# sjin09/himut

Hardware: AMD Instinct MI355X
Metric: Mbp scanned/sec at 30x CCS (himut call pileup scan) (higher is better)
Workload: dtype u8/int32 + f64 genotype tail; 1 GPU; chr20-sized contig (64444167 bp) 30x synthetic CCS per GPU, common-SNP + PoN filtering, reference chunking (323 chunks); reads_per_gpu=128888, read_bases_per_gpu=1932346823, parallelism=contig-per-gpu x1 + RCCL gather

## Files before the change

### himut_amd/csrc/himut_call.hip

```cpp
#include <hip/hip_runtime.h>

#include <string.h>
#include <rocprim/rocprim.hpp>

#include "himut_ctx.h"
#include "himut_kernels.h"
#include "himut_reads.h"

using namespace himut;

namespace himut {


namespace {

struct ParseSide {
    const Params* P = nullptr;
    uint32_t* bits = nullptr;
    int64_t nwords = 0;
    void* fill = nullptr;
    int64_t fill_slots = 0;
};

void ensure_group_plan(himut_ctx* c) {
// ... 252 lines not shown
    A.counts = c->call.d_dense_counts.as<uint32_t>(); A.bqsum = c->call.d_dense_bqsum.as<uint32_t>(); A.err = err;
    hipLaunchKernelGGL((k_pile_dense<PD_TP, PD_RB, PD_NT>), dim3((unsigned)T.n_tiles), dim3(PD_NT), 0, st, A);
}


void call_reserve_records(himut_ctx* c, CallPlan* P) {
    himut_ctx::Call& K = c->call;
    const int64_t nreserve = P->nreserve;
    K.d_recs.reserve((size_t)(nreserve + 1) * sizeof(himut_record));
    K.d_recs_out.reserve((size_t)(nreserve + 1) * sizeof(himut_record));
    if (P->ncap <= 0) return;
    K.d_keys.reserve((size_t)nreserve * 8); K.d_keys2.reserve((size_t)nreserve * 8);
    K.d_cands.reserve((size_t)nreserve * sizeof(Cand) + 256); K.d_cands2.reserve((size_t)nreserve * sizeof(Cand) + 256);
    K.d_emit.reserve((size_t)nreserve * 4);
    if (!c->chunks_in_order) {
        HCHECK(rocprim::radix_sort_pairs(nullptr, P->sort_tmp, K.d_keys.as<uint64_t>(), K.d_keys2.as<uint64_t>(), K.d_cands.as<uint64_t>(),
                                         K.d_cands2.as<uint64_t>(), (size_t)P->ncap, 0, 60, c->stream));
        c->d_tmp.reserve(P->sort_tmp + 256);
    }
    const unsigned nb = blocks_for(P->ncap, 256);
    K.d_logpart.reserve((size_t)nb * 16 * 4 + 64);
    K.d_pos.reserve((size_t)nb * 4 + 64);
}

int call_plan(himut_ctx* c, bool allow_spec, CallPlan* P) {
    himut_ctx::Call& K = c->call;
    P->T = upload_chunks(c, c->cstart, c->cend);
    P->phase = c->params.p.phase != 0;
    P->spec = allow_spec && c->chunks_in_order && K.cap_cand > 0 && K.cap_slots > 0 && P->T.positions > 0 && c->n > 0;
    alloc_derived(c);
    P->n4 = ((int64_t)P->T.positions * 2 + 15) / 16;
    P->mask_bytes = (size_t)P->n4 * 16;
    P->anyw = ((int64_t)P->T.positions + 31) / 32;
    P->mtiles = blocks_for(P->anyw, 256);
    const uint64_t mask_was = K.d_mask.gen;
    K.d_mask.reserve(P->mask_bytes + 64);
    const bool clear_mask = !K.mask_clean || mask_was != K.d_mask.gen;
    K.mask_clean = false;
    const uint64_t tcnt_was = K.d_tilecnt.gen;
    K.d_tilecnt.reserve((size_t)P->mtiles * 4 + 64);
    K.d_tileoff2.reserve((size_t)P->mtiles * 4 + 64);
    P->clear_all = clear_mask || tcnt_was != K.d_tilecnt.gen;
    if (P->phase && P->T.n > 65535) return fail(c, HIMUT_ERR_ARG, "--phase: more than 65,535 chunks in one contig (k_read_hap takes a chunk per grid row)");
    if (P->phase) c->d_hap.reserve((size_t)P->T.npairs + 64);
    P->F = front_plan(c, P->spec, K.cap_slots);
    if (P->mtiles > 65536u) {
        uint32_t* nul = nullptr;
        HCHECK(rocprim::exclusive_scan(nullptr, P->scan_tiles, nul, nul, 0u, (size_t)P->mtiles, rocprim::plus<uint32_t>(), c->stream));
    }
    c->d_tmp2.reserve(P->scan_tiles + 256);
    if (P->spec) {
        P->ncap = P->nreserve = K.cap_cand;
        call_reserve_records(c, P);
    }
    return HIMUT_OK;
}

int call_candidates(himut_ctx* c, CallPlan* P, const Chunks& C) {
    hipStream_t st = c->stream;
    himut_ctx::Call& K = c->call;
    Scalars* sc = c->d_scalars.as<Scalars>();
    uint32_t *tilecnt = K.d_tilecnt.as<uint32_t>(), *tileoff = K.d_tileoff2.as<uint32_t>();
    if (P->anyw > 0) {
        if (P->mtiles <= 65536u)
            hipLaunchKernelGGL(k_scan_small, dim3(1), dim3(1024), 0, st, tilecnt, tileoff, (int)P->mtiles);
        else
            HCHECK(rocprim::exclusive_scan(c->d_tmp2.p, P->scan_tiles, tilecnt, tileoff, 0u, (size_t)P->mtiles, rocprim::plus<uint32_t>(), st));
    }
    if (!P->spec) {
        uint32_t last_tcnt = 0, last_toff = 0;
        if (P->anyw > 0) {
            HCHECK(hipMemcpyAsync(&last_tcnt, tilecnt + (P->mtiles - 1), 4, hipMemcpyDeviceToHost, st));
            HCHECK(hipMemcpyAsync(&last_toff, tileoff + (P->mtiles - 1), 4, hipMemcpyDeviceToHost, st));
        }
        HCHECK(hipMemcpyAsync(c->h_scalars, sc, sizeof(Scalars), hipMemcpyDeviceToHost, st));
        HCHECK(hipStreamSynchronize(st));
        if (const int err = reinterpret_cast<const Scalars*>(c->h_scalars)->err) return check_device_err(c, err);
        P->ncap = (int64_t)last_toff + last_tcnt;
        P->nreserve = P->ncap + P->ncap / 4 + 1024;
        call_reserve_records(c, P);
    }
    if (P->ncap > 0) {
        const bool sorted = c->chunks_in_order;
        hipLaunchKernelGGL(k_mask_emit, dim3(P->mtiles), dim3(256), 0, st, K.d_posbits_c.as<uint32_t>(), (int64_t)P->T.positions,
                           K.d_mask.as<uint16_t>(), tileoff, C, (sorted ? K.d_cands2 : K.d_cands).as<Cand>(),
                           (sorted ? K.d_keys2 : K.d_keys).as<uint64_t>(), P->ncap, &sc->ncand, tilecnt);
        if (!sorted)
            HCHECK(rocprim::radix_sort_pairs(c->d_tmp.p, P->sort_tmp, K.d_keys.as<uint64_t>(), K.d_keys2.as<uint64_t>(), K.d_cands.as<uint64_t>(),
                                             K.d_cands2.as<uint64_t>(), (size_t)P->ncap, 0, 60, st));
    }
    stage_event(c, EV_EMIT, 2, st);
    return HIMUT_OK;
}

void call_eval(himut_ctx* c, const CallPlan& P, const Reads& R, const Derived& D, const Chunks& C, const Phase& H) {
    Scalars* sc = c->d_scalars.as<Scalars>();
    if (P.ncap > 0) {
        EvalArgs A;
        A.P = c->params;
        A.S = site_sets(c);
        A.lut = c->d_lut.as<GtLut>();
        A.cands = c->call.d_cands2.as<Cand>(); A.ncand = P.ncap; A.ncand_dev = &sc->ncand;
        A.R = R; A.D = D; A.C = C; A.H = H; A.X = P.F.X;
        A.colstore = c->call.d_colstore.as<uint16_t>(); A.nslots = (int64_t)P.F.slot_cap;
        A.recs = c->call.d_recs.as<himut_record>();
        A.err = &sc->err;
        hipLaunchKernelGGL(P.phase ? k_eval_columns<true> : k_eval_columns<false>, dim3(blocks_for(P.ncap, 256)), dim3(256), 0, c->stream, A);
    }
    stage_event(c, EV_SWEEP, 2, c->stream);
}

void call_finalize(himut_ctx* c, const CallPlan& P) {
    hipStream_t st = c->stream;
    himut_ctx::Call& K = c->call;
    Scalars* sc = c->d_scalars.as<Scalars>();
    if (P.ncap > 0) {
        const unsigned nb = blocks_for(P.ncap, 256);
        hipLaunchKernelGGL(k_finalize_flags, dim3(nb), dim3(256), 0, st, K.d_recs.as<himut_record>(), K.d_keys2.as<uint64_t>(),
                           &sc->ncand, P.ncap, K.d_emit.as<uint32_t>(), K.d_logpart.as<uint32_t>(),
                           c->d_ccs.as<uint8_t>(), c->n);
        hipLaunchKernelGGL(k_run_totals, dim3(1), dim3(1024), 0, st, P.ncap, K.d_blkoff.as<uint32_t>(), K.d_blkslots.as<uint32_t>(), P.F.nblk,
                           &sc->nrec, &sc->nslots, K.d_logpart.as<uint32_t>(), (int64_t)nb, sc->log, K.d_pos.as<uint32_t>());
        hipLaunchKernelGGL(k_compact, dim3(nb), dim3(256), 0, st, K.d_recs.as<himut_record>(), K.d_emit.as<uint32_t>(),
                           K.d_pos.as<uint32_t>(), &sc->ncand, P.ncap, K.d_recs_out.as<himut_record>());
    } else if (c->n > 0) {
        launch_count_flags(c, sc);
    }
}

int finish_run(himut_ctx* c, bool* overflow);

int do_run_once(himut_ctx* c, bool allow_spec, bool* overflow, bool defer) {
    *overflow = false;
    c->call.pending.active = false;
    if (int rc = check_scan_inputs(c)) return rc;
    HCHECK(hipSetDevice(c->device));
    c->call.h_recs_valid = false;
    c->call.n_out = 0;
    memset(c->call.log, 0, sizeof(c->call.log));
    memset(&c->stats, 0, sizeof(c->stats));
    c->params.unique_qnames = c->unique_qnames ? 1 : 0;

    CallPlan P;
    if (int rc = call_plan(c, allow_spec, &P)) return rc;
    const Reads R = make_reads(c);
    const Derived D = make_derived(c);
    const Chunks C = make_chunks(c, P.T.n);
    const Phase H = make_phase(c);
    front_decode(c, P.F, c->params, P.clear_all);
    if (P.phase && P.T.npairs > 0) launch_read_hap(c, R, D, C, H, P.T, c->d_scalars.as<Scalars>());
    stage_event(c, EV_HAP, 2, c->stream);
    if (int rc = front_capture(c, &P.F, C, H, c->params, c->call.d_mask.as<uint32_t>(), c->call.d_tilecnt.as<uint32_t>())) return rc;
    if (int rc = call_candidates(c, &P, C)) return rc;
    call_eval(c, P, R, D, C, H);
    call_finalize(c, P);
    front_tail(c, P.F);
    c->call.pending.active = true;
    c->call.pending.plan = P;
    if (defer) return HIMUT_OK;
    return finish_run(c, overflow);
}

int finish_run(himut_ctx* c, bool* overflow) {
    *overflow = false;
    const PendingRun Q = c->call.pending;
    c->call.pending.active = false;
    if (!Q.active) return HIMUT_OK;
    HCHECK(hipSetDevice(c->device));
// ... 177 lines not shown
```

### himut_amd/csrc/himut_kernels.h

```cpp
#pragma once

#include "himut_device.h"

namespace himut {

constexpr int EMIT_MAXC = 4;
constexpr int PROP_TAB_BITS = 11;

__device__ __forceinline__ void propose_read(const Reads& R, const Derived& D, const Chunks& C, const Phase& H, const Params& P,
                                             const int64_t r, const uint32_t bqs, const int e0, const int estride, const int gl,
                                             const int gsh, uint32_t* mask, uint32_t* tilecnt, uint8_t* ccs_flag,
                                             unsigned long long* s_seen) {
    auto propose = [&](const int64_t cell, const int bit) {
        if (s_seen) {
            const unsigned long long key = ((unsigned long long)cell << 4) | (unsigned long long)bit;
            const uint32_t h = (uint32_t)((key * 0x9E3779B97F4A7C15ull) >> (64 - PROP_TAB_BITS));
            if (atomicExch(&s_seen[h], key) == key) return;
        }
        const uint32_t m = (1u << bit) << ((cell & 1) ? 16 : 0);
        if (!(atomicOr(mask + (cell >> 1), m) & m)) atomicAdd(tilecnt + (cell >> MASK_TILE_SHIFT), 1u);
    };
#define GBALLOT(P) ((uint32_t)((__ballot(P) >> gsh) & 0xffffull))
    const ReadMeta M = D.meta[r];
    const int32_t qlen = R.qlen[r];
// ... 45 lines not shown
            for (int k = 0; k < EMIT_MAXC; k++) {
                if (rest) {
                    const int src = __ffs((int)rest) - 1;
                    rest &= rest - 1;
                    cc[k] = __shfl(rec.idx, src, 16); cst[k] = __shfl(rec.start, src, 16); cen[k] = __shfl(rec.end, src, 16);
                    cmo[k] = ((int64_t)__shfl((int)(rec.maskoff >> 32), src, 16) << 32) | (uint32_t)__shfl((int)rec.maskoff, src, 16);
                }
            }
        }
        if (nc == 0) live = false;
        else if (gl == 0) ccs_flag[qid] = 1;
    } else live = false;

    if (!live) return;
    const int32_t* mis = D.mis + M.segbase;
    const uint32_t* mq = D.mq + M.segbase;
    const double trim_start = floor(P.p.min_trim * (double)qlen);
    const double trim_end = ceil((1.0 - P.p.min_trim) * (double)qlen);
    const int64_t w = P.p.mismatch_window_size;
    for (int e = e0; e < nm; e += estride) {
        const uint32_t v = mq[e];
        const int32_t tp1 = mis[e];
        const int32_t mprev = e > 0 ? mis[e - 1] : -0x7fffffff - 1;
        const int32_t mnext = e + 1 < nm ? mis[e + 1] : 0x7fffffff;
        if (!(v & 16u)) continue;
        const int64_t q = v >> 5;
        if ((double)q < trim_start || (double)q > trim_end) continue;
        {
            int64_t qs = q - w, qe = q + w, ur, dr;
            if (qs < 0) { ur = w + qs; dr = w - qs; }
            else if (qe > qlen) { ur = w + (qe - qlen); dr = qlen - q; }
            else { ur = w; dr = w; }
            const int32_t ms = (int32_t)(tp1 - ur), me = (int32_t)(tp1 + dr);
            int lo = e, up = e + 1;
            if (mprev >= ms) { lo = e - 1; while (lo > 0 && mis[lo - 1] >= ms) lo--; }
            if (mnext <= me) { up = e + 2; while (up < nm && mis[up] <= me) up++; }
            if ((int64_t)(up - lo) - 1 > P.p.max_mismatch_count) continue;
        }
        const int bit = (int)(v & 15u);
        if (!overflow) {
#pragma unroll
            for (int k = 0; k < EMIT_MAXC; k++)
                if (cc[k] >= 0 && cst[k] <= tp1 && tp1 <= cen[k]) propose(cmo[k] + (tp1 - cst[k]), bit);
        } else {
            for (int64_t jj = hi - 1; jj >= 0 && C.rec[jj].pmaxend > ts; jj--) {
                const ChunkRec qr = C.rec[jj];
                if (qr.end <= ts || !(qr.start <= tp1 && tp1 <= qr.end)) continue;
                if (phase && H.hap[qr.pairbase + r] == HAP_NONE) continue;
                propose(qr.maskoff + (tp1 - qr.start), bit);
            }
        }
    }
#undef GBALLOT
}


struct CellCursor {
    int64_t ck, cbeg, cend;
    int32_t cstart;
};

__device__ __forceinline__ uint32_t cell_summary(const Chunks& C, const uint32_t* posbits, int64_t i, int64_t ncells, CellCursor& cur) {
    const int64_t c0 = i * 32;
    if (c0 >= ncells) return 0u;
    while (c0 >= cur.cend) { cur.ck++; cur.cbeg = cur.cend; cur.cend = C.maskoff[cur.ck + 1]; cur.cstart = C.start[cur.ck]; }
    if (c0 + 32 <= cur.cend) {
        const int64_t rp = (int64_t)cur.cstart + (c0 - cur.cbeg) - 1;
        if (rp < 0) return posbits[0] << 1;
        const uint32_t lo = posbits[rp >> 5], hi = posbits[(rp >> 5) + 1];
        const int sh = (int)(rp & 31);
        return sh ? ((lo >> sh) | (hi << (32 - sh))) : lo;
    }
    uint32_t w = 0;
    CellCursor t = cur;
    for (int b = 0; b < 32 && c0 + b < ncells; b++) {
        const int64_t c = c0 + b;
        while (c >= t.cend) { t.ck++; t.cbeg = t.cend; t.cend = C.maskoff[t.ck + 1]; t.cstart = C.start[t.ck]; }
        const int64_t rp = (int64_t)t.cstart + (c - t.cbeg) - 1;
        if (rp >= 0 && ((posbits[rp >> 5] >> (rp & 31)) & 1u)) w |= 1u << b;
    }
    return w;
}

__global__ void __launch_bounds__(256) k_mask_emit(const uint32_t* posbits, int64_t ncells, uint16_t* mask16, const uint32_t* tileoff,
                                                   Chunks C, Cand* cands, uint64_t* keys, int64_t cap, unsigned long long* total,
                                                   uint32_t* tilecnt) {
    __shared__ int s_w[4];
    const int lane = threadIdx.x & 63, wv = threadIdx.x >> 6;
    const int64_t i = (int64_t)blockIdx.x * 256 + threadIdx.x;
    if (threadIdx.x == 0) tilecnt[blockIdx.x] = 0;
    const MaskTile mt = C.mtile[blockIdx.x];
    CellCursor cur = {mt.ck0, mt.off0, mt.off1, mt.start0};
    uint32_t w = cell_summary(C, posbits, i, ncells, cur);
    int c = 0;
    for (uint32_t x = w; x; x &= x - 1) c += __popc((uint32_t)mask16[i * 32 + (__ffs((int)x) - 1)]);
    const int incl = wave_incl_add(c, lane);
    if (lane == 63) s_w[wv] = incl;
    __syncthreads();
    if (blockIdx.x == gridDim.x - 1 && threadIdx.x == 0)
        *total = (unsigned long long)tileoff[blockIdx.x] + (unsigned long long)(s_w[0] + s_w[1] + s_w[2] + s_w[3]);
    if (!c) return;
    int64_t slot = (int64_t)tileoff[blockIdx.x] + (incl - c);
#pragma unroll
    for (int k = 0; k < 4; k++) if (k < wv) slot += s_w[k];
    int64_t ck = cur.ck;
    int64_t cbeg = cur.cbeg, cend_ = cur.cend;
    int32_t cstart = cur.cstart;
    while (w) {
        const int b = __ffs((int)w) - 1; w &= w - 1;
        const int64_t cell = i * 32 + b;
        const uint32_t m = mask16[cell];
        if (!m) continue;
        mask16[cell] = 0;
        while (cell >= cend_) { ck++; cbeg = cend_; cend_ = C.maskoff[ck + 1]; cstart = C.start[ck]; }
        const int32_t tpos = cstart + (int32_t)(cell - cbeg);
#pragma unroll
        for (int rk = 0; rk < 16; rk++) {
            const int ra = (0x1230 >> (4 * (rk >> 2))) & 15, aa = (0x1230 >> (4 * (rk & 3))) & 15;
            const int bit = (ra << 2) | aa;
            if ((m >> bit) & 1u) {
                if (slot < cap) {
                    Cand cd; cd.tpos = tpos; cd.chunk_bit = ((uint32_t)ck << 4) | (uint32_t)bit;
                    cands[slot] = cd;
                    keys[slot] = ((uint64_t)(uint32_t)tpos << 28) | ((uint64_t)ck << 4) | (uint64_t)rk;
                }
                slot++;
            }
        }
    }
}
struct BlockCount {
    const uint32_t* bits;
    const int32_t *winlo, *winhi;
    __host__ __device__ uint2 operator()(int64_t b) const {
        const uint4* wp = reinterpret_cast<const uint4*>(bits + (b << 3));
        const uint4 x = wp[0], y = wp[1];
        const uint32_t cnt = (uint32_t)(__builtin_popcount(x.x) + __builtin_popcount(x.y) + __builtin_popcount(x.z) + __builtin_popcount(x.w) +
                                        __builtin_popcount(y.x) + __builtin_popcount(y.y) + __builtin_popcount(y.z) + __builtin_popcount(y.w));
        const unsigned long long s = ((unsigned long long)cnt * (unsigned long long)(uint32_t)(winhi[b] - winlo[b]) + 15ULL) & ~15ULL;
        return make_uint2(cnt, (uint32_t)s);
    }
};

__device__ __forceinline__ void block_counts(const BlockCount& F, int64_t b, uint32_t& cnt, uint32_t& nr, unsigned long long& slots) {
    const uint4* wp = reinterpret_cast<const uint4*>(F.bits + (b << 3));
    const uint4 x = wp[0], y = wp[1];
    cnt = (uint32_t)(__popc(x.x) + __popc(x.y) + __popc(x.z) + __popc(x.w) + __popc(y.x) + __popc(y.y) + __popc(y.z) + __popc(y.w));
    nr = (uint32_t)(F.winhi[b] - F.winlo[b]);
    slots = ((unsigned long long)cnt * (unsigned long long)nr + 15ULL) & ~15ULL;
}
__device__ __forceinline__ void wg_sum2(uint32_t& a, unsigned long long& b, uint32_t* s_a, unsigned long long* s_b) {
#pragma unroll
    for (int d = 32; d > 0; d >>= 1) { a += __shfl_xor(a, d, 64); b += __shfl_xor(b, d, 64); }
    const int wv = threadIdx.x >> 6;
    __syncthreads();
    if ((threadIdx.x & 63) == 0) { s_a[wv] = a; s_b[wv] = b; }
    __syncthreads();
    a = s_a[0] + s_a[1] + s_a[2] + s_a[3];
    b = s_b[0] + s_b[1] + s_b[2] + s_b[3];
}
__global__ void __launch_bounds__(256) k_block_sums(BlockCount F, int64_t nblk, int per, uint4* part) {
    __shared__ uint32_t s_a[4];
    __shared__ unsigned long long s_b[4];
    const int64_t b0 = ((int64_t)blockIdx.x * 256 + threadIdx.x) * per;
    uint32_t c = 0;
    unsigned long long s = 0;
    for (int k = 0; k < per; k++)
        if (b0 + k < nblk) { uint32_t cnt, nr; unsigned long long sl; block_counts(F, b0 + k, cnt, nr, sl); c += cnt; s += sl; }
    wg_sum2(c, s, s_a, s_b);
    if (threadIdx.x == 0) part[blockIdx.x] = make_uint4(c, 0u, (uint32_t)s, (uint32_t)(s >> 32));
}
__global__ void __launch_bounds__(256) k_block_table3(BlockCount F, int64_t nblk, int per, const uint4* part, BlockTab* bt,
                                                      uint32_t* blkoff, uint32_t* blkslots, int* err) {
    __shared__ uint32_t s_a[4];
    __shared__ unsigned long long s_b[4];
    uint32_t pc = 0;
    unsigned long long ps = 0;
    for (int w = threadIdx.x; w < (int)blockIdx.x; w += 256) {
        const uint4 v = part[w];
        pc += v.x; ps += (unsigned long long)v.z | ((unsigned long long)v.w << 32);
    }
    wg_sum2(pc, ps, s_a, s_b);
    const int64_t b0 = ((int64_t)blockIdx.x * 256 + threadIdx.x) * per;
    uint32_t tc = 0;
    unsigned long long ts = 0;
    for (int k = 0; k < per; k++)
        if (b0 + k < nblk) { uint32_t cnt, nr; unsigned long long sl; block_counts(F, b0 + k, cnt, nr, sl); tc += cnt; ts += sl; }
    uint32_t ic = tc;
    unsigned long long is = ts;
    const int lane = threadIdx.x & 63, wv = threadIdx.x >> 6;
#pragma unroll
    for (int d = 1; d < 64; d <<= 1) {
        const uint32_t uc = __shfl_up(ic, d, 64);
        const unsigned long long us = __shfl_up(is, d, 64);
        if (lane >= d) { ic += uc; is += us; }
    }
    __syncthreads();
    if (lane == 63) { s_a[wv] = ic; s_b[wv] = is; }
    __syncthreads();
    uint32_t rc = pc + ic - tc;
    unsigned long long rs = ps + is - ts;
    for (int w = 0; w < wv; w++) { rc += s_a[w]; rs += s_b[w]; }
    bool deep = false;
    for (int k = 0; k < per; k++) {
        const int64_t b = b0 + k;
        if (b >= nblk) break;
        uint32_t cnt, nr;
        unsigned long long sl;
        block_counts(F, b, cnt, nr, sl);
        BlockTab t;
        t.lo = F.winlo[b]; t.ncnt = nr | (cnt << 22); t.boff = (uint32_t)rs; t.ufirst = rc;
// ... 296 lines not shown
                    const int64_t slot = (int64_t)t.z + (int64_t)(r - (int32_t)t.x) * (int64_t)(t.y >> 22) + (int64_t)(u - t.w);
                    if ((uint64_t)slot < (uint64_t)A.nslots) A.colstore[slot] = (uint16_t)val;
                }
            }
        };
        while (true) {
            const int32_t hiP = min(tB, covB);
            int32_t e = 0x7fffffff;
            if (i_list + lane < n_list) e = lbase + (int32_t)list[i_list + lane];
            const bool act = e < hiP;
            const int bn = (int)__popcll(__ballot(act));
            if (bn) {
                batch(act, (uint32_t)e, u_list + (uint32_t)(i_list + lane), lane_val(e, bn - 1));
                i_list += bn;
            }
            if (bn == 64) continue;
            if (tB <= covB || covB > tend) break;
            __builtin_amdgcn_wave_barrier();
            refill();
        }
#pragma unroll
        for (int i = 0; i < CPD; i++) ta[i] = ta[i + 1];
        ta[CPD] = ta_next;
    };

    for (int k = 0; k < nwin; k += CPD) {
        window(ba0, bb0, sq0, bt0r, k);
        window(ba1, bb1, sq1, bt1r, k + 1);
        if constexpr (CPD > 2) window(ba2, bb2, sq2, bt2r, k + 2);
        if constexpr (CPD > 3) window(ba3, bb3, sq3, bt3r, k + 3);
    }
    {
        if (A.bqsum) {
#pragma unroll
            for (int d = 32; d > 0; d >>= 1) qsum += __shfl_down(qsum, d, 64);
            if (lane == 0) A.bqsum[r] = qsum;
            if (R.nonacgt && uni((int)R.nonacgt[r])) {
                int64_t lo_ = 0, hi_ = A.C.n;
                while (lo_ < hi_) { const int64_t m_ = (lo_ + hi_) >> 1; if (A.C.rec[m_].start < tend) lo_ = m_ + 1; else hi_ = m_; }
                if (lo_ > 0 && A.C.rec[lo_ - 1].pmaxend > tstart && __ballot(!aligned_bases_ok(R, gsegs, ns, qo, lane, 64)))
                    set_err(const_cast<int*>(A.err), HIMUT_ERR_BASE);
            }
            if (A.mask) propose_read(R, A.D, A.C, A.H, A.P, r, uni(qsum), lane, 64, lane & 15, lane & 48, A.mask, A.tilecnt, A.ccs_flag, nullptr);
        }
    }
#undef CAP_ISSUE
#undef CAP_SEGWIN
#undef CAP_LANDED4
#undef CAP_LANDED2
}

__global__ void __launch_bounds__(256, HIMUT_CAP_WAVES) k_stream_capture(CaptureArgs A) { capture_wave(A); }


struct EvalArgs {
    Params P;
    SiteSets S;
    const GtLut* lut;
    const Cand* cands;
    int64_t ncand;
    const unsigned long long* ncand_dev;
    Reads R;
    Derived D;
    Chunks C;
    Phase H;
    PosIndex X;
    const uint16_t* colstore;
    int64_t nslots;
    himut_record* recs;
    int* err;
};

#ifndef HIMUT_EVAL_WAVES
#define HIMUT_EVAL_WAVES 4
#endif
#ifndef HIMUT_EVAL_BATCH
#define HIMUT_EVAL_BATCH 8
#endif
template <bool PHASE>
__global__ void __launch_bounds__(256, HIMUT_EVAL_WAVES) k_eval_columns(EvalArgs A) {
    __shared__ double s_lut[3 * 256];
    __shared__ double s_prior[4];
    const int tid = threadIdx.x;
    for (int i = tid; i < 3 * 256; i += 256) s_lut[i] = A.lut->t[i >> 8][i & 255];
    if (tid < 4) s_prior[tid] = A.lut->prior[tid];
    __syncthreads();
    const int64_t j = (int64_t)blockIdx.x * blockDim.x + tid;
    if (j >= dev_count(A.ncand_dev, A.ncand) || *A.err) return;
    const Cand cd = A.cands[j];
    const int32_t tpos = cd.tpos;
    const int chunk = (int)(cd.chunk_bit >> 4);
    const int ref = (int)((cd.chunk_bit >> 2) & 3), alt = (int)(cd.chunk_bit & 3);
    const int32_t rpos = tpos - 1;
    const uint32_t u = pos_rank(A.X, rpos);
    const BlockTab bt = A.X.bt[rpos >> 8];
    const uint32_t n = bt.ncnt & BT_N_MASK, stride = bt.ncnt >> 22;
    const int32_t lo = bt.lo;
    const uint16_t* col = A.colstore + ((int64_t)bt.boff + (int64_t)(u - bt.ufirst));
    if (n && (int64_t)bt.boff + (int64_t)(u - bt.ufirst) + (int64_t)(n - 1) * (int64_t)stride >= A.nslots) return;
    const int min_bq = A.P.p.min_bq;
    const int32_t cs_ = A.C.start[chunk];
    const bool edge = rpos <= cs_;

    uint32_t cnt[6] = {0, 0, 0, 0, 0, 0};
    uint32_t bqs[4] = {0, 0, 0, 0};
    GtSums S;
#pragma unroll
    for (int b = 0; b < 4; b++) { S[0][b] = 0.0; S[1][b] = 0.0; S[2][b] = 0.0; }
    uint32_t ref_count = 0, alt_count = 0, alt_hi = 0, h0_ref = 0, h1_ref = 0, som0 = 0, som1 = 0;
    double R0 = 0.0, R1 = 0.0, R2 = 0.0, A0 = 0.0, A1 = 0.0, A2 = 0.0;
    uint32_t Rq = 0, Aq = 0;
    int bad = 0;
    constexpr int EB = HIMUT_EVAL_BATCH;
    for (uint32_t i0 = 0; i0 < n; i0 += EB) {
      uint32_t vv[EB];
#pragma unroll
      for (int k = 0; k < EB; k++) vv[k] = (i0 + k < n) ? (uint32_t)col[(int64_t)(i0 + k) * stride] : (uint32_t)CELL_EMPTY;
#pragma unroll
      for (int k = 0; k < EB; k++) {
        const uint32_t i = i0 + k;
        const uint32_t v = vv[k];
        const uint32_t cell = v & 7u;
        if ((v & 15u) == CELL_EMPTY) continue;
        int32_t tend = 0;
        if (edge || PHASE) {
            tend = A.R.tend[lo + (int32_t)i];
            if (edge && !(tend > cs_)) continue;
        }
        if (v & CELL_INS) cnt[4]++;
        if (cell < 4) {
            const uint32_t q = v >> 8;
            if (q == 0) bad |= 1 << HIMUT_ERR_BQ0;
            const double vh = s_lut[q], vt = s_lut[256 + q], ve = s_lut[512 + q];
            if ((int)cell == ref) {
                ref_count++; Rq += q;
                R0 = R0 + vh; R1 = R1 + vt; R2 = R2 + ve;
            } else if ((int)cell == alt) {
                alt_count++; Aq += q; if ((int)q >= min_bq) alt_hi++;
                A0 = A0 + vh; A1 = A1 + vt; A2 = A2 + ve;
            } else {
#pragma unroll
                for (int b = 0; b < 4; b++) {
                    if ((int)cell == b) {
                        cnt[b]++; bqs[b] += q;
                        S[0][b] = S[0][b] + vh;
                        S[1][b] = S[1][b] + vt;
                        S[2][b] = S[2][b] + ve;
                    }
                }
            }
            if (PHASE) {
                uint32_t hp = HAP_NONE;
                if (tend > rpos + 1 && ((int)cell == ref || (int)cell == alt))
                    hp = A.H.hap[A.C.pairoff[chunk] + ((int64_t)(lo + (int32_t)i) - A.C.rlo[chunk])];
                if ((int)cell == ref) { if (hp == HAP_0) h0_ref++; else if (hp == HAP_1) h1_ref++; }
                if ((int)cell == alt) { if (hp == HAP_0) som0 = 1; else if (hp == HAP_1) som1 = 1; }
            }
        } else if (cell == CELL_DEL) cnt[5]++;
        else if (cell == CELL_OTHER) bad |= 1 << HIMUT_ERR_BASE;
      }
    }

#pragma unroll
    for (int b = 0; b < 4; b++) {
        if (b == ref) { cnt[b] = ref_count; bqs[b] = Rq; S[0][b] = R0; S[1][b] = R1; S[2][b] = R2; }
        if (b == alt) { cnt[b] = alt_count; bqs[b] = Aq; S[0][b] = A0; S[1][b] = A1; S[2][b] = A2; }
    }
    const Genotype gt = genotype(S, s_prior, ref);
    const int gq = gt.gq;
    int g0 = (int)HIMUT_GT_B1(gt.best), g1 = (int)HIMUT_GT_B2(gt.best);
    const int state = gt_state_of(g0, g1, ref);
    if (g0 != ref && ((g0 == ref) + (g1 == ref)) == 1) { int tmp = g0; g0 = g1; g1 = tmp; }

    const uint32_t depth = cnt[0] + cnt[1] + cnt[2] + cnt[3] + cnt[5];
    bool germ;
    if (state == 1) germ = (g0 == ref && g1 == alt);
    else if (state == 2) {
        uint32_t c0 = 0, c1 = 0;
#pragma unroll
        for (int b = 0; b < 4; b++) { if (g0 == b) c0 = cnt[b]; if (g1 == b) c1 = cnt[b]; }
        germ = ((cnt[0] + cnt[1] + cnt[2] + cnt[3]) == (c0 + c1)) && (alt == g0 || alt == g1);
    } else if (state == 3) germ = (ref_count == 0) && (g0 == alt && g1 == alt);
    else germ = (alt == g0);

    int status = 255;
    int32_t ps = -1;
    uint32_t flags = 0;
    if (germ) flags = REC_GERM;
    else if (state == 1) status = HIMUT_ST_HET;
    else if (state == 2) status = HIMUT_ST_HETALT;
    else if (state == 3) status = HIMUT_ST_HOMALT;
    else if (cnt[5] != 0 || cnt[4] != 0) status = HIMUT_ST_INDEL;
    else {
        const uint64_t key = ((uint64_t)(uint32_t)tpos << 4) | ((uint64_t)ref << 2) | (uint64_t)alt;
        if (gq < A.P.p.min_gq) status = HIMUT_ST_LOWGQ;
        else if (alt_hi == 0) status = HIMUT_ST_LOWBQ;
        else {
            const SiteSets& St = A.S;
            const bool site_maybe = (int64_t)tpos < St.nposbits && ((St.posbits[tpos >> 5] >> (tpos & 31)) & 1u);
            if (site_maybe && key_in(St.pon, St.npon, key)) status = HIMUT_ST_PON;
            else if (site_maybe && key_in(St.com, St.ncom, key)) status = HIMUT_ST_COMSNP;
            else if (!((int64_t)ref_count >= A.P.p.min_ref_count && (int64_t)alt_count >= A.P.p.min_alt_count)) status = HIMUT_ST_LOWDEPTH;
            else if ((int64_t)depth > A.P.p.md_threshold) status = HIMUT_ST_HIGHDEPTH;
            else if (PHASE) {
                if (!A.P.unique_qnames) {
                    h0_ref = h1_ref = som0 = som1 = 0;
                    const int32_t p1 = rpos + 1;
                    const BlockTab b1 = A.X.bt[min((int64_t)(p1 >> 8), A.X.nblk - 1)];
                    const uint32_t n1 = b1.ncnt & BT_N_MASK;
                    for (uint32_t jj = 0; jj < n1; jj++) {
                        const int64_t jr = (int64_t)b1.lo + jj;
                        if (!(A.R.tstart[jr] <= p1 && A.R.tend[jr] > p1) || (A.D.rflag[jr] & RF_SECONDARY)) continue;
                        const int32_t qj = A.R.qid[jr];
                        bool in_wt = false, in_alt = false;
                        for (uint32_t i = 0; i < n; i++) {
                            const uint32_t v = (uint32_t)col[(int64_t)i * stride];
                            const int cv = (int)(v & 7u);
                            if ((v & 15u) == CELL_EMPTY || (cv != ref && cv != alt)) continue;
                            if (edge && !(A.R.tend[lo + (int32_t)i] > cs_)) continue;
                            if (A.R.qid[lo + (int32_t)i] != qj) continue;
                            if (cv == ref) in_wt = true; else in_alt = true;
                        }
                        if (!in_wt && !in_alt) continue;
                        uint32_t hp = HAP_NONE;
                        if (jr >= A.C.rlo[chunk] && jr < A.C.rhi[chunk]) hp = A.H.hap[A.C.pairoff[chunk] + (jr - A.C.rlo[chunk])];
                        if (in_wt) { if (hp == HAP_0) h0_ref++; else if (hp == HAP_1) h1_ref++; }
                        else { if (hp == HAP_0) som0 = 1; else if (hp == HAP_1) som1 = 1; }
                    }
                }
                if ((int64_t)h0_ref >= A.P.p.min_hap_count && (int64_t)h1_ref >= A.P.p.min_hap_count && (som0 + som1) == 1) {
                    status = HIMUT_ST_PASS; ps = cs_;
                } else status = HIMUT_ST_UNPHASED;
            } else status = HIMUT_ST_PASS;
        }
    }
    uint4 w0, w1, w2, w3;
    w0.x = (uint32_t)tpos; w0.y = (uint32_t)chunk; w0.z = (uint32_t)ps; w0.w = (uint32_t)gq;
    w1.x = (uint32_t)allele2char(ref) | ((uint32_t)allele2char(alt) << 8) | ((uint32_t)allele2char(g0) << 16) | ((uint32_t)allele2char(g1) << 24);
    w1.y = (uint32_t)(status & 255) | ((uint32_t)state << 8) | (flags << 16);
    w1.z = cnt[0]; w1.w = cnt[1];
    w2.x = cnt[2]; w2.y = cnt[3]; w2.z = cnt[4]; w2.w = cnt[5];
    w3.x = bqs[0]; w3.y = bqs[1]; w3.z = bqs[2]; w3.w = bqs[3];
    uint4* dst = reinterpret_cast<uint4*>(A.recs + j);
    dst[0] = w0; dst[1] = w1; dst[2] = w2; dst[3] = w3;
    if (bad) atomicOr(A.err, bad);
}


struct TileInfo {
    int32_t chunk;
    int32_t p0;
    int32_t npos;
    int32_t nwin;
    int64_t lo;
    int64_t outbase;
};

template <int TP>
__global__ void __launch_bounds__(256) k_tile_index(Reads R, Chunks C, const int64_t* tileoff, int64_t n_tiles, TileInfo* out) {
    const int64_t tile = (int64_t)blockIdx.x * blockDim.x + threadIdx.x;
    if (tile >= n_tiles) return;
    const int64_t c = upper_bound(tileoff, (int64_t)0, C.n + 1, tile) - 1;
    const int32_t cs_ = C.start[c], ce_ = C.end[c];
    const int64_t local = (tile - tileoff[c]) * TP;
    TileInfo t;
    t.chunk = (int32_t)c;
    t.p0 = (int32_t)(cs_ - 1 + local);
    const int32_t p1 = (int32_t)min((int64_t)t.p0 + TP, (int64_t)ce_);
    t.npos = p1 - t.p0;
    const int64_t rlo = C.rlo[c], rhi = C.rhi[c];
    const int64_t hi = lower_bound(R.tstart, rlo, rhi, p1);
    const int64_t lo = lower_bound(R.prefmax_tend, rlo, hi, t.p0);
    t.lo = lo;
    t.nwin = (int32_t)(hi - lo);
    t.outbase = C.maskoff[c] + local;
    out[tile] = t;
}

struct DenseArgs {
    Reads R;
    Derived D;
    Chunks C;
// ... 115 lines not shown
                        if (pc.flags & SEG_DEL) {
                            cell = (cell & ~(nm & 0x7777777777777777ULL)) | (nm & 0x5555555555555555ULL);
                        } else {
                            const int64_t o = qo + pc.qa + (cov ? (gx + a - pc.x0) : 0);
                            const uint8_t* sp = R.seq + (o >> 1);
                            uint32_t w32;
                            __builtin_memcpy(&w32, sp, 4);
                            const uint32_t extra = sp[4];
                            uint64_t l;
                            __builtin_memcpy(&l, R.bq + o, 8);
                            uint64_t w = w32;
                            w = ((w & 0x0f0f0f0f0f0f0f0fULL) << 4) | ((w >> 4) & 0x0f0f0f0f0f0f0f0fULL);
                            if (o & 1) w = (w >> 4) | ((uint64_t)(extra >> 4) << 28);
                            const uint64_t codes = nib16_to_cells(w) << (4 * aa);
                            if (codes & nm & 0x4444444444444444ULL) bad |= 1 << HIMUT_ERR_BASE;
                            cell = (cell & ~(nm & 0x7777777777777777ULL)) | (codes & nm);
                            const uint64_t bm = ((bb >= 8) ? ~0ULL : ((1ULL << (8 * bb)) - 1ULL)) & ~((1ULL << (8 * aa)) - 1ULL);
                            bqw |= (l << (8 * aa)) & bm;
                        }
                    }
                } else {
                    const int64_t rr = T.lo + s_rowread[i];
                    const Seg* segs = D.segs + seg_base(R, rr);
                    const int ns = D.nseg[rr];
                    for (int j = 0; j < PPL; j++) {
                        const int32_t pp = p0 + gx + j;
                        for (int q = 0; q < ns; q++) {
                            const Seg sg = segs[q];
                            if (sg.t0 > pp) break;
                            if (pp == sg.t0 && (sg.flags & SEG_INS)) cell |= 8ULL << (4 * j);
                            if (pp < sg.t0 + sg.len) {
                                uint64_t code;
                                if (sg.flags & SEG_DEL) code = CELL_DEL;
                                else {
                                    const int64_t o = qo + sg.q0 + (pp - sg.t0);
                                    code = (uint64_t)nib2allele(nib_at(R.seq, o));
                                    bqw |= (uint64_t)R.bq[o] << (8 * j);
                                }
                                cell = (cell & ~(7ULL << (4 * j))) | (code << (4 * j));
                            }
                        }
                    }
                }
                *reinterpret_cast<uint32_t*>(&s_cell[i * (TP / 2) + lane * 4]) = (uint32_t)cell;
                *reinterpret_cast<uint64_t*>(&s_bq[i * TP + lane * 8]) = bqw;
            }
            __syncthreads();
#pragma unroll
            for (int d = 0; d < DPT; d++) {
                const int x = tid + d * NT;
                if (x < T.npos) {
                    for (int i = 0; i < nb; i++) {
                        const uint32_t cb = (s_cell[i * (TP / 2) + (x >> 1)] >> (4 * (x & 1))) & 15;
                        if (cb == CELL_EMPTY) continue;
                        if (cb & CELL_INS) dcnt[d][4]++;
                        const int a = cb & 7;
                        if (a < 4) {
                            const uint32_t q = s_bq[i * TP + x];
#pragma unroll
                            for (int b = 0; b < 4; b++) if (a == b) { dcnt[d][b]++; dbq[d][b] += q; }
                        } else if (a == CELL_DEL) dcnt[d][5]++;
                        else if (a == CELL_OTHER) bad |= 1 << HIMUT_ERR_BASE;
                    }
                }
            }
            __syncthreads();
        }
    }
#pragma unroll
    for (int d = 0; d < DPT; d++) {
        const int x = tid + d * NT;
        if (x < T.npos) {
            const int64_t o = T.outbase + x;
#pragma unroll
            for (int k = 0; k < 6; k++) A.counts[o * 6 + k] = dcnt[d][k];
#pragma unroll
            for (int k = 0; k < 4; k++) A.bqsum[o * 4 + k] = dbq[d][k];
        }
    }
    if (bad) atomicOr(A.err, bad);
}


__device__ __forceinline__ bool seen_in_earlier_chunk(const himut_record* recs, const uint64_t* keys, int64_t i, int64_t n) {
    const uint64_t tp = keys[i] >> 28;
    const bool first = i == 0 || (keys[i - 1] >> 28) != tp;
    if (first) return false;
    const uint64_t mych = (keys[i] >> 4) & 0xffffff;
    int64_t j = i;
    while (j > 0 && (keys[j - 1] >> 28) == tp) j--;
    bool seen = false;
    while (j < n && (keys[j] >> 28) == tp) {
        const uint64_t ch = (keys[j] >> 4) & 0xffffff;
        if (ch == mych) break;
        bool nongerm = false;
        int64_t k = j;
        while (k < n && (keys[k] >> 28) == tp && ((keys[k] >> 4) & 0xffffff) == ch) {
            if (!(recs[k].flags & REC_GERM)) nongerm = true;
            k++;
        }
        if (nongerm) seen = true;
        j = k;
    }
    return seen;
}

__global__ void __launch_bounds__(256) k_finalize_flags(himut_record* recs, const uint64_t* keys, const unsigned long long* n_dev,
                                                        int64_t cap, uint32_t* emit, uint32_t* logpart, const uint8_t* ccs,
                                                        int64_t nreads) {
    __shared__ unsigned int s_log[16];
    if (threadIdx.x < 16) s_log[threadIdx.x] = 0;
    __syncthreads();
    const int64_t i = (int64_t)blockIdx.x * blockDim.x + threadIdx.x;
    {
        unsigned int f = 0;
        for (int64_t j = i; j < nreads; j += (int64_t)gridDim.x * 256) f += ccs[j];
#pragma unroll
        for (int d = 32; d > 0; d >>= 1) f += __shfl_xor(f, d, 64);
        if ((threadIdx.x & 63) == 0 && f) atomicAdd(&s_log[0], f);
    }
    const int64_t n = dev_count(n_dev, cap);
    if (i >= n && i < cap) emit[i] = 0;
    int slot = -1, slot2 = -1;
    bool counted = false, emitted = false;
    if (i < n) {
        himut_record& rec = recs[i];
        uint32_t e = 0;
        const bool suppressed = seen_in_earlier_chunk(recs, keys, i, n);
        if (!suppressed) {
            counted = true;
            if (rec.flags & REC_GERM) {
                if (rec.gt_state == 1) slot = 2;
                else if (rec.gt_state == 2) slot = 3;
                else if (rec.gt_state == 3) slot = 4;
            } else {
                const int st = rec.status;
                if (st == HIMUT_ST_HET || st == HIMUT_ST_HETALT || st == HIMUT_ST_HOMALT) slot = 5;
                else if (st == HIMUT_ST_INDEL) slot = 7;
                else {
                    slot = 6;
                    if (st == HIMUT_ST_LOWGQ) slot2 = 8;
                    else if (st == HIMUT_ST_LOWBQ) slot2 = 9;
                    else if (st == HIMUT_ST_PON) slot2 = 10;
                    else if (st == HIMUT_ST_COMSNP) slot2 = 11;
                    else if (st == HIMUT_ST_HIGHDEPTH) slot2 = 12;
                    else if (st == HIMUT_ST_LOWDEPTH) slot2 = 13;
                    else slot2 = 14;
                }
                e = 1;
                if (st == HIMUT_ST_HETALT && i > 0) {
                    const uint64_t m = ~(uint64_t)3;
                    if ((keys[i - 1] & m) == (keys[i] & m)) {
                        const himut_record& prev = recs[i - 1];
                        if (prev.status == HIMUT_ST_HETALT && !(prev.flags & REC_GERM)) { e = 0; rec.flags |= REC_DUP; }
                    }
                }
            }
        }
        emit[i] = e;
        emitted = e != 0;
    }
    const int lane = threadIdx.x & 63;
    {
        const unsigned long long b = __ballot(counted);
        if (lane == 0 && b) atomicAdd(&s_log[1], (unsigned int)__popcll(b));
        const unsigned long long be = __ballot(emitted);
        if (lane == 0 && be) atomicAdd(&s_log[15], (unsigned int)__popcll(be));
    }
    if (__ballot(slot >= 0 || slot2 >= 0)) {
#pragma unroll
        for (int k = 2; k < 15; k++) {
            const unsigned long long b = __ballot(slot == k || slot2 == k);
            if (lane == 0 && b) atomicAdd(&s_log[k], (unsigned int)__popcll(b));
        }
    }
    __syncthreads();
    if (threadIdx.x < 16) logpart[(int64_t)blockIdx.x * 16 + threadIdx.x] = s_log[threadIdx.x];
}

__global__ void __launch_bounds__(256) k_compact(const himut_record* recs, const uint32_t* emit, const uint32_t* wgoff,
                                                 const unsigned long long* n_dev, int64_t cap, himut_record* out) {
    __shared__ uint32_t s_w[4];
    const int64_t i = (int64_t)blockIdx.x * blockDim.x + threadIdx.x;
    const bool e = i < dev_count(n_dev, cap) && emit[i] != 0;
    const unsigned long long b = __ballot(e);
    const int lane = threadIdx.x & 63, wv = threadIdx.x >> 6;
    if (lane == 0) s_w[wv] = (uint32_t)__popcll(b);
    __syncthreads();
    if (!e) return;
    uint32_t pos = wgoff[blockIdx.x] + (uint32_t)__popcll(b & ((1ull << lane) - 1ull));
    for (int w = 0; w < wv; w++) pos += s_w[w];
    const uint4* src = reinterpret_cast<const uint4*>(recs + i);
    uint4 a = src[0], bb = src[1], c = src[2], d = src[3];
    bb.y &= 0xff00ffffu;
    uint4* dst = reinterpret_cast<uint4*>(out + pos);
    dst[0] = a; dst[1] = bb; dst[2] = c; dst[3] = d;
}

__global__ void __launch_bounds__(1024) k_run_totals(int64_t cap, const uint32_t* blkoff, const uint32_t* blkslots, int64_t nblk,
                                                     unsigned long long* nrec, unsigned long long* nslots, const uint32_t* logpart,
                                                     int64_t nparts, unsigned long long* log, uint32_t* wgoff) {
    __shared__ unsigned long long s_log[16];
    __shared__ uint32_t s_w[16];
    if (threadIdx.x < 16) s_log[threadIdx.x] = 0;
    __syncthreads();
    const int q = threadIdx.x & 3;
    unsigned long long a0 = 0, a1 = 0, a2 = 0, a3 = 0;
#pragma unroll 4
    for (int64_t b = threadIdx.x >> 2; b < nparts; b += 256) {
        const uint4 v = *reinterpret_cast<const uint4*>(logpart + b * 16 + q * 4);
        a0 += v.x; a1 += v.y; a2 += v.z; a3 += v.w;
    }
#pragma unroll
    for (int d = 4; d < 64; d <<= 1) {
        a0 += __shfl_xor(a0, d, 64); a1 += __shfl_xor(a1, d, 64); a2 += __shfl_xor(a2, d, 64); a3 += __shfl_xor(a3, d, 64);
    }
    if ((threadIdx.x & 63) < 4) {
        atomicAdd(&s_log[q * 4 + 0], a0); atomicAdd(&s_log[q * 4 + 1], a1);
        atomicAdd(&s_log[q * 4 + 2], a2); atomicAdd(&s_log[q * 4 + 3], a3);
    }
    const int per = (int)((nparts + 1023) / 1024);
    const int64_t p0 = (int64_t)threadIdx.x * per;
    uint32_t t = 0;
    for (int k = 0; k < per; k++) if (p0 + k < nparts) t += logpart[(p0 + k) * 16 + 15];
    uint32_t inc = t;
    const int lane = threadIdx.x & 63, wv = threadIdx.x >> 6;
#pragma unroll
    for (int d = 1; d < 64; d <<= 1) { const uint32_t u = __shfl_up(inc, d, 64); if (lane >= d) inc += u; }
    if (lane == 63) s_w[wv] = inc;
    __syncthreads();
    uint32_t run = inc - t;
    for (int w = 0; w < wv; w++) run += s_w[w];
    for (int k = 0; k < per; k++) if (p0 + k < nparts) { wgoff[p0 + k] = run; run += logpart[(p0 + k) * 16 + 15]; }
    if (threadIdx.x < 15) log[threadIdx.x] = s_log[threadIdx.x];
    if (threadIdx.x == 0) {
        *nrec = cap > 0 ? s_log[15] : 0ull;
        *nslots = nblk > 0 ? (unsigned long long)blkoff[nblk - 1] + blkslots[nblk - 1] : 0ull;
// ... 5 lines not shown
```

Measured before the change: 68650 Mbp/s.

## Restructure mask emit to one wave per tile and hoist loads in eval/finalize

k_mask_emit now assigns one wave per mask tile, with each lane covering four 32-cell words. The wave scan alone yields the tile offset, which removes the shared-memory cross-wave reduction and the __syncthreads. Mask reads are batched eight at a time so loads are in flight together, and the first batch is reused in the emit pass. In the eval and finalize kernels, global loads (block table, rank, chunk start, site word, keys, packed record word) are issued before the barrier or the branches to hide latency. The changes rely on the record layout, reading status, gt_state and flags from the second uint4, and add register pressure.

After: 66980 Mbp/s. -2.4%, worse.

```diff
diff --git a/himut_amd/csrc/himut_call.hip b/himut_amd/csrc/himut_call.hip
--- a/himut_amd/csrc/himut_call.hip
+++ b/himut_amd/csrc/himut_call.hip
@@ -358,8 +358,9 @@
     }
     if (P->ncap > 0) {
         const bool sorted = c->chunks_in_order;
-        hipLaunchKernelGGL(k_mask_emit, dim3(P->mtiles), dim3(256), 0, st, K.d_posbits_c.as<uint32_t>(), (int64_t)P->T.positions,
-                           K.d_mask.as<uint16_t>(), tileoff, C, (sorted ? K.d_cands2 : K.d_cands).as<Cand>(),
+        hipLaunchKernelGGL(k_mask_emit, dim3(blocks_for((int64_t)P->mtiles, EMIT_WG_TILES)), dim3(64 * EMIT_WG_TILES), 0, st,
+                           K.d_posbits_c.as<uint32_t>(), (int64_t)P->T.positions, K.d_mask.as<uint16_t>(), tileoff,
+                           (int64_t)P->mtiles, C, (sorted ? K.d_cands2 : K.d_cands).as<Cand>(),
                            (sorted ? K.d_keys2 : K.d_keys).as<uint64_t>(), P->ncap, &sc->ncand, tilecnt);
         if (!sorted)
             HCHECK(rocprim::radix_sort_pairs(c->d_tmp.p, P->sort_tmp, K.d_keys.as<uint64_t>(), K.d_keys2.as<uint64_t>(), K.d_cands.as<uint64_t>(),
diff --git a/himut_amd/csrc/himut_kernels.h b/himut_amd/csrc/himut_kernels.h
--- a/himut_amd/csrc/himut_kernels.h
+++ b/himut_amd/csrc/himut_kernels.h
@@ -151,35 +151,83 @@
     return w;
 }
 
-__global__ void __launch_bounds__(256) k_mask_emit(const uint32_t* posbits, int64_t ncells, uint16_t* mask16, const uint32_t* tileoff,
-                                                   Chunks C, Cand* cands, uint64_t* keys, int64_t cap, unsigned long long* total,
-                                                   uint32_t* tilecnt) {
-    __shared__ int s_w[4];
-    const int lane = threadIdx.x & 63, wv = threadIdx.x >> 6;
-    const int64_t i = (int64_t)blockIdx.x * 256 + threadIdx.x;
-    if (threadIdx.x == 0) tilecnt[blockIdx.x] = 0;
-    const MaskTile mt = C.mtile[blockIdx.x];
+constexpr int EMIT_LANE_WORDS = 4;
+constexpr int EMIT_WG_TILES = 4;
+constexpr int EMIT_BATCH = 8;
+static_assert(EMIT_LANE_WORDS * 32 * 64 == MASK_TILE_CELLS, "a wave covers one mask tile");
+
+__device__ __forceinline__ int emit_next_bit(unsigned long long& x0, unsigned long long& x1) {
+    const bool up = x0 == 0ull;
+    const unsigned long long x = up ? x1 : x0;
+    const int b = x ? (up ? 64 : 0) + (__ffsll((long long)x) - 1) : -1;
+    const unsigned long long rest = x & (x - 1ull);
+    x0 = up ? 0ull : rest;
+    x1 = up ? rest : x1;
+    return b;
+}
+
+__global__ void __launch_bounds__(64 * EMIT_WG_TILES) k_mask_emit(const uint32_t* posbits, int64_t ncells, uint16_t* mask16,
+                                                                  const uint32_t* tileoff, int64_t mtiles, Chunks C, Cand* cands,
+                                                                  uint64_t* keys, int64_t cap, unsigned long long* total,
+                                                                  uint32_t* tilecnt) {
+    const int lane = threadIdx.x & 63;
+    const int64_t tile = (int64_t)blockIdx.x * EMIT_WG_TILES + (threadIdx.x >> 6);
+    if (tile >= mtiles) return;
+    const MaskTile mt = C.mtile[tile];
+    const uint32_t toff = tileoff[tile];
+    if (lane == 0) tilecnt[tile] = 0;
+    const int64_t i0 = tile * (MASK_TILE_CELLS / 32) + lane * EMIT_LANE_WORDS;
+    const int64_t c0 = i0 * 32;
     CellCursor cur = {mt.ck0, mt.off0, mt.off1, mt.start0};
-    uint32_t w = cell_summary(C, posbits, i, ncells, cur);
+    uint32_t w[EMIT_LANE_WORDS];
+#pragma unroll
+    for (int k = 0; k < EMIT_LANE_WORDS; k++) w[k] = 0u;
+    if (c0 < ncells) {
+        while (c0 >= cur.cend) { cur.ck++; cur.cbeg = cur.cend; cur.cend = C.maskoff[cur.ck + 1]; cur.cstart = C.start[cur.ck]; }
+        const int64_t rp = (int64_t)cur.cstart + (c0 - cur.cbeg) - 1;
+        if (c0 + 32 * EMIT_LANE_WORDS <= cur.cend && rp >= 0) {
+            uint32_t pw[EMIT_LANE_WORDS + 1];
+#pragma unroll
+            for (int k = 0; k <= EMIT_LANE_WORDS; k++) pw[k] = posbits[(rp >> 5) + k];
+            const int sh = (int)(rp & 31);
+#pragma unroll
+            for (int k = 0; k < EMIT_LANE_WORDS; k++) w[k] = sh ? ((pw[k] >> sh) | (pw[k + 1] << (32 - sh))) : pw[k];
+        } else {
+            CellCursor t = cur;
+#pragma unroll
+            for (int k = 0; k < EMIT_LANE_WORDS; k++) w[k] = cell_summary(C, posbits, i0 + k, ncells, t);
+        }
+    }
+    const unsigned long long s0 = (unsigned long long)w[0] | ((unsigned long long)w[1] << 32);
+    const unsigned long long s1 = (unsigned long long)w[2] | ((unsigned long long)w[3] << 32);
+    unsigned long long x0 = s0, x1 = s1;
+    uint32_t mv[EMIT_BATCH];
+#pragma unroll
+    for (int k = 0; k < EMIT_BATCH; k++) {
+        const int b = emit_next_bit(x0, x1);
+        mv[k] = b >= 0 ? (uint32_t)mask16[c0 + b] : 0u;
+    }
     int c = 0;
-    for (uint32_t x = w; x; x &= x - 1) c += __popc((uint32_t)mask16[i * 32 + (__ffs((int)x) - 1)]);
+#pragma unroll
+    for (int k = 0; k < EMIT_BATCH; k++) c += __popc(mv[k]);
+    while (x0 | x1) {
+        uint32_t mr[EMIT_BATCH];
+#pragma unroll
+        for (int k = 0; k < EMIT_BATCH; k++) {
+            const int b = emit_next_bit(x0, x1);
+            mr[k] = b >= 0 ? (uint32_t)mask16[c0 + b] : 0u;
+        }
+#pragma unroll
+        for (int k = 0; k < EMIT_BATCH; k++) c += __popc(mr[k]);
+    }
     const int incl = wave_incl_add(c, lane);
-    if (lane == 63) s_w[wv] = incl;
-    __syncthreads();
-    if (blockIdx.x == gridDim.x - 1 && threadIdx.x == 0)
-        *total = (unsigned long long)tileoff[blockIdx.x] + (unsigned long long)(s_w[0] + s_w[1] + s_w[2] + s_w[3]);
+    if (tile == mtiles - 1 && lane == 63) *total = (unsigned long long)toff + (unsigned long long)incl;
     if (!c) return;
-    int64_t slot = (int64_t)tileoff[blockIdx.x] + (incl - c);
-#pragma unroll
-    for (int k = 0; k < 4; k++) if (k < wv) slot += s_w[k];
+    int64_t slot = (int64_t)toff + (incl - c);
     int64_t ck = cur.ck;
     int64_t cbeg = cur.cbeg, cend_ = cur.cend;
     int32_t cstart = cur.cstart;
-    while (w) {
-        const int b = __ffs((int)w) - 1; w &= w - 1;
-        const int64_t cell = i * 32 + b;
-        const uint32_t m = mask16[cell];
-        if (!m) continue;
+    auto emit_cell = [&](const int64_t cell, const uint32_t m) {
         mask16[cell] = 0;
         while (cell >= cend_) { ck++; cbeg = cend_; cend_ = C.maskoff[ck + 1]; cstart = C.start[ck]; }
         const int32_t tpos = cstart + (int32_t)(cell - cbeg);
@@ -196,6 +244,16 @@
                 slot++;
             }
         }
+    };
+    x0 = s0; x1 = s1;
+    for (int k = 0; x0 | x1; k++) {
+        const int64_t cell = c0 + emit_next_bit(x0, x1);
+        uint32_t m = 0;
+        if (k < EMIT_BATCH) {
+#pragma unroll
+            for (int kk = 0; kk < EMIT_BATCH; kk++) m = kk == k ? mv[kk] : m;
+        } else m = mask16[cell];
+        if (m) emit_cell(cell, m);
     }
 }
 struct BlockCount {
@@ -658,24 +716,36 @@
     __shared__ double s_lut[3 * 256];
     __shared__ double s_prior[4];
     const int tid = threadIdx.x;
-    for (int i = tid; i < 3 * 256; i += 256) s_lut[i] = A.lut->t[i >> 8][i & 255];
-    if (tid < 4) s_prior[tid] = A.lut->prior[tid];
-    __syncthreads();
     const int64_t j = (int64_t)blockIdx.x * blockDim.x + tid;
-    if (j >= dev_count(A.ncand_dev, A.ncand) || *A.err) return;
-    const Cand cd = A.cands[j];
+    const double l0 = A.lut->t[0][tid], l1 = A.lut->t[1][tid], l2 = A.lut->t[2][tid];
+    double pr = 0.0;
+    if (tid < 4) pr = A.lut->prior[tid];
+    Cand cd; cd.tpos = 1; cd.chunk_bit = 0u;
+    if (j < A.ncand) cd = A.cands[j];
+    const bool live = j < dev_count(A.ncand_dev, A.ncand) && !*A.err;
     const int32_t tpos = cd.tpos;
     const int chunk = (int)(cd.chunk_bit >> 4);
     const int ref = (int)((cd.chunk_bit >> 2) & 3), alt = (int)(cd.chunk_bit & 3);
     const int32_t rpos = tpos - 1;
-    const uint32_t u = pos_rank(A.X, rpos);
-    const BlockTab bt = A.X.bt[rpos >> 8];
+    BlockTab bt; bt.lo = 0; bt.ncnt = 0u; bt.boff = 0u; bt.ufirst = 0u;
+    uint32_t rk = 0, site_word = 0;
+    int32_t cs_ = 0;
+    if (live) {
+        bt = A.X.bt[rpos >> 8];
+        rk = pos_rank_in_block(A.X.bits, rpos);
+        cs_ = A.C.start[chunk];
+        if ((int64_t)tpos < A.S.nposbits) site_word = A.S.posbits[tpos >> 5];
+    }
+    s_lut[tid] = l0; s_lut[256 + tid] = l1; s_lut[512 + tid] = l2;
+    if (tid < 4) s_prior[tid] = pr;
+    __syncthreads();
+    if (!live) return;
+    const uint32_t u = bt.ufirst + rk;
     const uint32_t n = bt.ncnt & BT_N_MASK, stride = bt.ncnt >> 22;
     const int32_t lo = bt.lo;
     const uint16_t* col = A.colstore + ((int64_t)bt.boff + (int64_t)(u - bt.ufirst));
     if (n && (int64_t)bt.boff + (int64_t)(u - bt.ufirst) + (int64_t)(n - 1) * (int64_t)stride >= A.nslots) return;
     const int min_bq = A.P.p.min_bq;
-    const int32_t cs_ = A.C.start[chunk];
     const bool edge = rpos <= cs_;
 
     uint32_t cnt[6] = {0, 0, 0, 0, 0, 0};
@@ -773,7 +843,7 @@
         else if (alt_hi == 0) status = HIMUT_ST_LOWBQ;
         else {
             const SiteSets& St = A.S;
-            const bool site_maybe = (int64_t)tpos < St.nposbits && ((St.posbits[tpos >> 5] >> (tpos & 31)) & 1u);
+            const bool site_maybe = (int64_t)tpos < St.nposbits && ((site_word >> (tpos & 31)) & 1u);
             if (site_maybe && key_in(St.pon, St.npon, key)) status = HIMUT_ST_PON;
             else if (site_maybe && key_in(St.com, St.ncom, key)) status = HIMUT_ST_COMSNP;
             else if (!((int64_t)ref_count >= A.P.p.min_ref_count && (int64_t)alt_count >= A.P.p.min_alt_count)) status = HIMUT_ST_LOWDEPTH;
@@ -1055,11 +1125,12 @@
 }
 
 
-__device__ __forceinline__ bool seen_in_earlier_chunk(const himut_record* recs, const uint64_t* keys, int64_t i, int64_t n) {
-    const uint64_t tp = keys[i] >> 28;
-    const bool first = i == 0 || (keys[i - 1] >> 28) != tp;
+__device__ __forceinline__ bool seen_in_earlier_chunk(const himut_record* recs, const uint64_t* keys, int64_t i, int64_t n,
+                                                      const uint64_t key, const uint64_t keyp) {
+    const uint64_t tp = key >> 28;
+    const bool first = i == 0 || (keyp >> 28) != tp;
     if (first) return false;
-    const uint64_t mych = (keys[i] >> 4) & 0xffffff;
+    const uint64_t mych = (key >> 4) & 0xffffff;
     int64_t j = i;
     while (j > 0 && (keys[j - 1] >> 28) == tp) j--;
     bool seen = false;
@@ -1085,6 +1156,14 @@
     if (threadIdx.x < 16) s_log[threadIdx.x] = 0;
     __syncthreads();
     const int64_t i = (int64_t)blockIdx.x * blockDim.x + threadIdx.x;
+    const int64_t n = dev_count(n_dev, cap);
+    uint64_t key = 0, keyp = 0;
+    uint4 w1 = make_uint4(0u, 0u, 0u, 0u);
+    if (i < n) {
+        key = keys[i];
+        if (i > 0) keyp = keys[i - 1];
+        w1 = reinterpret_cast<const uint4*>(recs + i)[1];
+    }
     {
         unsigned int f = 0;
         for (int64_t j = i; j < nreads; j += (int64_t)gridDim.x * 256) f += ccs[j];
@@ -1092,22 +1171,21 @@
         for (int d = 32; d > 0; d >>= 1) f += __shfl_xor(f, d, 64);
         if ((threadIdx.x & 63) == 0 && f) atomicAdd(&s_log[0], f);
     }
-    const int64_t n = dev_count(n_dev, cap);
     if (i >= n && i < cap) emit[i] = 0;
     int slot = -1, slot2 = -1;
     bool counted = false, emitted = false;
     if (i < n) {
-        himut_record& rec = recs[i];
+        const int st = (int)(w1.y & 255u), gt_state = (int)((w1.y >> 8) & 255u);
+        const uint32_t flags = (w1.y >> 16) & 255u;
         uint32_t e = 0;
-        const bool suppressed = seen_in_earlier_chunk(recs, keys, i, n);
+        const bool suppressed = seen_in_earlier_chunk(recs, keys, i, n, key, keyp);
         if (!suppressed) {
             counted = true;
-            if (rec.flags & REC_GERM) {
-                if (rec.gt_state == 1) slot = 2;
-                else if (rec.gt_state == 2) slot = 3;
-                else if (rec.gt_state == 3) slot = 4;
+            if (flags & REC_GERM) {
+                if (gt_state == 1) slot = 2;
+                else if (gt_state == 2) slot = 3;
+                else if (gt_state == 3) slot = 4;
             } else {
-                const int st = rec.status;
                 if (st == HIMUT_ST_HET || st == HIMUT_ST_HETALT || st == HIMUT_ST_HOMALT) slot = 5;
                 else if (st == HIMUT_ST_INDEL) slot = 7;
                 else {
@@ -1123,9 +1201,9 @@
                 e = 1;
                 if (st == HIMUT_ST_HETALT && i > 0) {
                     const uint64_t m = ~(uint64_t)3;
-                    if ((keys[i - 1] & m) == (keys[i] & m)) {
+                    if ((keyp & m) == (key & m)) {
                         const himut_record& prev = recs[i - 1];
-                        if (prev.status == HIMUT_ST_HETALT && !(prev.flags & REC_GERM)) { e = 0; rec.flags |= REC_DUP; }
+                        if (prev.status == HIMUT_ST_HETALT && !(prev.flags & REC_GERM)) { e = 0; recs[i].flags = (uint8_t)(flags | REC_DUP); }
                     }
                 }
             }
```
